# gsanya/orbslam2_NMI

Measured on AMD Instinct MI355X. Metric: pose-candidate NMI evals/sec (640x480, 256 bins), one blocking nmi_search_grid call per step incl. its 8-byte read-back (SURVEY.md 8d's definition); beside the W warm-up steps an untimed clock warm-up of clock_warmup_ms = 200 ms precedes the timed region, higher is better.
Workload: dtype u8

## Files before the change

orbslam2_nmi_amd/csrc/nmi_grid_device.h:

```cpp
#pragma once
#include <hip/hip_runtime.h>
#include <stdint.h>

#include "nmi_kernels.h"
#include "nmi_device.h"

namespace nmi {

namespace {

constexpr int kBlock = NMI_BLOCK_THREADS;
constexpr int kWaves = kBlock / 64;
constexpr int kBins = 256;
constexpr int kWords = kBins * kBins / 2;
constexpr int kRowStride = 129;
constexpr int kJointWords = kBins * kRowStride;
constexpr int kOvfCap = 1024;
constexpr int kRowsPerWave = kBins / kWaves;
constexpr int kLdsTable = 4096;
constexpr int kSide = 8;


struct Lds {
    uint32_t joint[kJointWords];
// ... 30 lines not shown
template <bool BG, bool SHIFTED>
__device__ __forceinline__ void add_pixel(Lds &lds, int par, uint32_t d1, uint32_t d2, int shift)
{
    if (!BG && (d1 == 0 || d2 == 0)) return;
    if (SHIFTED) {
        d1 >>= shift;
        d2 >>= shift;
    }
    const uint32_t word = joint_word(d1, d2), val = joint_inc(d2);
    const uint32_t old = __hip_atomic_fetch_add(&lds.joint[word], val, __ATOMIC_RELAXED, __HIP_MEMORY_SCOPE_WORKGROUP);
    const uint32_t field = val * 0xFFFFu;
    if (__builtin_expect((old & field) == field, 0)) record_wrap(lds, par, word, val, old);
}

__device__ __forceinline__ bool side_add(Lds &lds, int par, uint32_t d1, uint32_t d2, uint32_t weight)
{
    const uint32_t key1 = ((d1 << 8) | d2) + 1u;
    for (int e = 0; e < kSide; ++e) {
        const uint32_t old = atomicCAS(&lds.side_key[par][e], 0u, key1);
        if (old == 0u || old == key1) {
            atomicAdd(&lds.side_cnt[par][e], weight);
            return true;
        }
    }
    return false;
}

template <bool BG, bool SHIFTED, int HIST>
__device__ __forceinline__ bool fold_flat_chunk(Lds &lds, int par, const uint32_t (&r)[4], const uint32_t (&w)[4], int shift)
{
    const uint32_t rb = r[0] & 0xFFu, wb = w[0] & 0xFFu;
    const bool flat = r[0] == r[1] && r[1] == r[2] && r[2] == r[3] && w[0] == w[1] && w[1] == w[2] && w[2] == w[3] &&
                      r[0] == rb * 0x01010101u && w[0] == wb * 0x01010101u;
    if (!__all(flat)) return false;
    uint32_t d1 = rb, d2 = wb;
    const bool skip = !BG && (d1 == 0 || d2 == 0);
    if (SHIFTED) {
        d1 >>= shift;
        d2 >>= shift;
    }
    const uint32_t key = (d1 << 8) | d2;
    const uint32_t key0 = __builtin_amdgcn_readfirstlane(key);
    const bool skip0 = __builtin_amdgcn_readfirstlane((uint32_t)skip) != 0;
    const uint32_t word = joint_word(d1, d2), high = d2 >> 7;
    uint32_t weight = 16;
    bool issue = !skip;
    if (__all(key == key0 && skip == skip0)) {
        const unsigned long long active = __ballot(1);
        weight = 16u * (uint32_t)__popcll(active);
        issue = issue && (__lane_id() == (uint32_t)__ffsll((long long)active) - 1u);
        if (issue && side_add(lds, par, d1, d2, weight)) issue = false;
    }
    if (issue) {
        const uint32_t inc = high ? weight << 16 : weight;
        if (HIST == 2) {
            (void)__hip_atomic_fetch_add(&lds.joint[word], inc, __ATOMIC_RELAXED, __HIP_MEMORY_SCOPE_WORKGROUP);
        } else {
            const uint32_t old = __hip_atomic_fetch_add(&lds.joint[word], inc, __ATOMIC_RELAXED, __HIP_MEMORY_SCOPE_WORKGROUP);
            const uint32_t field_old = high ? old >> 16 : old & 0xFFFFu;
            if (field_old + weight > 0xFFFFu) record_wrap(lds, par, word, high ? 0x10000u : 1u, high ? old : (old | 0xFFFFu));
        }
    }
    return true;
}

template <bool BG, bool SHIFTED, int HIST, bool FOLD>
__device__ __forceinline__ void add_chunk(Lds &lds, int par, const uint4 &rv, const uint4 &wv, int shift, bool try_flat)
{
    const uint32_t r[4] = {rv.x, rv.y, rv.z, rv.w};
    const uint32_t w[4] = {wv.x, wv.y, wv.z, wv.w};
    if (HIST == 0) {
#pragma unroll
        for (int q = 0; q < 4; ++q)
#pragma unroll
            for (int j = 0; j < 4; ++j)
                add_pixel<BG, SHIFTED>(lds, par, (r[q] >> (8 * j)) & 0xFFu, (w[q] >> (8 * j)) & 0xFFu, shift);
        return;
    }
    if (FOLD && HIST != 0 && try_flat) {
        if (__builtin_expect(flat_hint(rv, wv), 0)) {
            if (fold_flat_chunk<BG, SHIFTED, HIST>(lds, par, r, w, shift)) return;
        }
    }
    if (HIST == 2 && BG && !SHIFTED) {
        char *const base = reinterpret_cast<char *>(lds.joint);
        const uint32_t row_bytes = kRowStride * 4, k_ffff = 0xFFFFu;
#pragma unroll
        for (int q = 0; q < 4; ++q) {
#pragma unroll
            for (int j = 0; j < 4; ++j) {
                uint32_t a1, c, addr, hi, val;
                if (j == 0)
                    asm("v_mul_u32_u24_sdwa %0, %1, %2 dst_sel:DWORD dst_unused:UNUSED_PAD src0_sel:BYTE_0 src1_sel:DWORD" : "=v"(a1) : "v"(r[q]), "s"(row_bytes));
                else if (j == 1)
                    asm("v_mul_u32_u24_sdwa %0, %1, %2 dst_sel:DWORD dst_unused:UNUSED_PAD src0_sel:BYTE_1 src1_sel:DWORD" : "=v"(a1) : "v"(r[q]), "s"(row_bytes));
                else if (j == 2)
                    asm("v_mul_u32_u24_sdwa %0, %1, %2 dst_sel:DWORD dst_unused:UNUSED_PAD src0_sel:BYTE_2 src1_sel:DWORD" : "=v"(a1) : "v"(r[q]), "s"(row_bytes));
                else
                    asm("v_mul_u32_u24_sdwa %0, %1, %2 dst_sel:DWORD dst_unused:UNUSED_PAD src0_sel:BYTE_3 src1_sel:DWORD" : "=v"(a1) : "v"(r[q]), "s"(row_bytes));
                c = __builtin_amdgcn_ubfe(w[q], 8 * j, 7);
                asm("v_lshl_add_u32 %0, %1, 2, %2" : "=v"(addr) : "v"(c), "v"(a1));
                hi = __builtin_amdgcn_ubfe(w[q], 8 * j + 7, 1);
                asm("v_mad_u32_u24 %0, %1, %2, 1" : "=v"(val) : "v"(hi), "s"(k_ffff));
                (void)__hip_atomic_fetch_add(reinterpret_cast<uint32_t *>(base + addr), val, __ATOMIC_RELAXED, __HIP_MEMORY_SCOPE_WORKGROUP);
            }
        }
        return;
    }
    uint32_t old[16];
    uint32_t any = 0;
#pragma unroll
    for (int q = 0; q < 4; ++q) {
#pragma unroll
// ... 13 lines not shown
                    old[q * 4 + j] = __hip_atomic_fetch_add(&lds.joint[word], val, __ATOMIC_RELAXED, __HIP_MEMORY_SCOPE_WORKGROUP);
            }
        }
    }
    if (HIST == 1) {
#pragma unroll
        for (int q = 0; q < 4; ++q)
#pragma unroll
            for (int j = 0; j < 4; ++j) {
                uint32_t d2 = (w[q] >> (8 * j)) & 0xFFu;
                if (SHIFTED) d2 >>= shift;
                const uint32_t notfield = (d2 & 128u) ? 0x0000FFFFu : 0xFFFF0000u;
                const uint32_t t = old[q * 4 + j] | notfield;
                any = t > any ? t : any;
            }
        if (__builtin_expect(any == 0xFFFFFFFFu, 0)) {
#pragma unroll
            for (int q = 0; q < 4; ++q)
#pragma unroll
                for (int j = 0; j < 4; ++j) {
                    uint32_t d1 = (r[q] >> (8 * j)) & 0xFFu, d2 = (w[q] >> (8 * j)) & 0xFFu;
                    const bool skip = !BG && (d1 == 0 || d2 == 0);
                    if (SHIFTED) {
                        d1 >>= shift;
                        d2 >>= shift;
                    }
                    const uint32_t val = joint_inc(d2), field = val * 0xFFFFu;
                    if (!skip && (old[q * 4 + j] & field) == field) record_wrap(lds, par, joint_word(d1, d2), val, old[q * 4 + j]);
                }
        }
    }
}

#ifndef NMI_SLAB_SHARES_QUALIFIER
#define NMI_SLAB_SHARES_QUALIFIER __constant__ const
#endif
NMI_SLAB_SHARES_QUALIFIER uint32_t slab_cum[2][kWaves + 1] = {
    {0, 7048, 14096, 21145, 28193, 34369, 40546, 46722, 52899, 55010, 57120, 59231, 61342, 62390, 63439, 64487, 65536},
    {0, 5934, 12896, 19858, 26820, 33147, 39384, 45621, 51859, 54448, 56633, 58818, 61003, 62222, 63327, 64431, 65536},
};

template <bool BG, bool SHIFTED, int HIST, int NT, bool FOLD = true, bool ROWS = false, bool SLABS = false>
__device__ __forceinline__ void histogram_phase(Lds &lds, int par, const GridArgs &a, const uint8_t *__restrict__ render,
                                                const uint8_t *__restrict__ warped, int tid, int c_first, int c_end, bool later = false)
{
    static_assert(!SLABS || NT == kBlock, "slabs are per wavefront of a whole workgroup");
    if (ROWS || a.vec_ok) {
        const int nchunks = c_end;
        const int row_rem = ROWS ? a.width - (a.chunks_per_row << 4) : 0;
        auto ldw = [&](int c) {
            if (ROWS) return *reinterpret_cast<const uint4 *>(warped + (((uint32_t)c << 4) + (uint32_t)__mul24((int)__umulhi((uint32_t)c, a.cpr_magic), row_rem)));
            return *reinterpret_cast<const uint4 *>(warped + ((uint32_t)c << 4));
        };
        auto ldr = [&](int c) {
            const int y = (int)__umulhi((uint32_t)c, a.cpr_magic);
            if (ROWS) {
                const int ry = a.flip ? a.height - 1 - y : y;
                return *reinterpret_cast<const uint4 *>(render + (((uint32_t)(__mul24(y, a.flip_row) + c + a.flip_base) << 4) + (uint32_t)__mul24(ry, row_rem)));
            }
            return *reinterpret_cast<const uint4 *>(render + ((uint32_t)(__mul24(y, a.flip_row) + c + a.flip_base) << 4));
        };
        constexpr bool kHint = FOLD && HIST != 0;
        const bool try_flat = kHint && !(a.phase_mask & 4);
        constexpr int kStep = SLABS ? 64 : NT;
        int base = c_first, stop = nchunks, first = c_first + tid;
        if (SLABS) {
            const uint32_t v = __builtin_amdgcn_readfirstlane((uint32_t)tid >> 6), n = (uint32_t)(nchunks - c_first);
            const uint32_t *cum = slab_cum[later ? 1 : 0];
            base = c_first + (int)(((unsigned long long)n * cum[v]) >> 16);
            stop = c_first + (int)(((unsigned long long)n * cum[v + 1]) >> 16);
            first = base + (tid & 63);
        }
        const int last = SLABS ? max(stop, c_first + 1) - 1 : nchunks - 1;
        const int iters = (stop - base + kStep - 1) / kStep;
        int resume = (HIST == 1 && kHint) ? first : -1;
        if (resume < 0) {
            int ch = first;
            int c0 = min(ch, last);
            uint4 wa = ldw(c0), ra = ldr(c0), wb, rb;
            for (int it = 0; it < iters; it += 2) {
                const int c1 = min(ch + kStep, last);
                wb = ldw(c1);
                rb = ldr(c1);
                if (kHint && __builtin_expect(flat_hint(ra, wa), 0)) {
                    resume = ch;
                    break;
                }
                if (ch < stop) add_chunk<BG, SHIFTED, HIST, false>(lds, par, ra, wa, a.shift, false);
                const int c2 = min(ch + 2 * kStep, last);
                wa = ldw(c2);
                ra = ldr(c2);
                if (kHint && __builtin_expect(flat_hint(rb, wb), 0)) {
                    resume = ch + kStep;
                    break;
                }
                if (ch + kStep < stop) add_chunk<BG, SHIFTED, HIST, false>(lds, par, rb, wb, a.shift, false);
                ch += 2 * kStep;
            }
        }
        if (resume >= 0) {
            int c = min(resume, last);
            uint4 wc = ldw(c), rc = ldr(c);
#pragma unroll 1
            for (int ch = resume; ch < stop; ch += kStep) {
                const int cn = min(ch + kStep, last);
                const uint4 wn = ldw(cn), rn = ldr(cn);
                add_chunk<BG, SHIFTED, HIST, true>(lds, par, rc, wc, a.shift, try_flat);
                wc = wn;
                rc = rn;
            }
        }
        if (ROWS && row_rem > 0) {
            const int x0 = a.chunks_per_row << 4, n = a.height * row_rem;
            for (int t = tid; t < n; t += NT) {
                const int y = t / row_rem, x = x0 + t - y * row_rem;
                const int ry = a.flip ? (a.height - 1 - y) : y;
                uint32_t d1 = render[ry * a.width + x], d2 = warped[y * a.width + x];
                if (HIST == 2) {
                    if (BG || (d1 != 0 && d2 != 0)) {
                        if (SHIFTED) {
                            d1 >>= a.shift;
                            d2 >>= a.shift;
                        }
                        (void)__hip_atomic_fetch_add(&lds.joint[joint_word(d1, d2)], joint_inc(d2), __ATOMIC_RELAXED, __HIP_MEMORY_SCOPE_WORKGROUP);
                    }
                } else {
                    add_pixel<BG, SHIFTED>(lds, par, d1, d2, a.shift);
                }
            }
        }
    } else {
        for (int pos = tid; pos < a.npix; pos += NT) {
            const int y = pos / a.width;
            const int x = pos - y * a.width;
            const int ry = a.flip ? (a.height - 1 - y) : y;
            if (HIST == 2) {
                uint32_t d1 = render[ry * a.width + x], d2 = warped[pos];
                if (BG || (d1 != 0 && d2 != 0)) {
                    if (SHIFTED) {
                        d1 >>= a.shift;
                        d2 >>= a.shift;
                    }
                    (void)__hip_atomic_fetch_add(&lds.joint[joint_word(d1, d2)], joint_inc(d2), __ATOMIC_RELAXED,
// ... 11 lines not shown
    return c ? table[c] : 0.0f;
}
__device__ __forceinline__ float term_lds(const Lds &lds, const float *__restrict__ table, uint32_t c)
{
    float t = lds.table[c < (uint32_t)kLdsTable ? c : 0u];
    if (__builtin_expect(c >= (uint32_t)kLdsTable, 0)) t = table[c];
    return t;
}

static_assert(kWaves == 16 && (kWaves * kRowStride) % 32 == 16, "rows kWaves apart must fall on opposite halves of the 32 banks");
__device__ __forceinline__ int decode_row(int wave, int pass, int r) { return wave + 4 * kWaves * pass + kWaves * r; }
__device__ __forceinline__ bool in_decode_pass(uint32_t d1, int wave, int pass)
{
    return (d1 % (uint32_t)kWaves) == (uint32_t)wave && (d1 / (uint32_t)(4 * kWaves)) == (uint32_t)pass;
}
__device__ __forceinline__ uint32_t decode_word(int d1, int i, int k) { return (uint32_t)(d1 * kRowStride + i + 16 * k); }

__device__ __forceinline__ void apply_wraps(const Lds &lds, int par, uint32_t novf, uint32_t word, uint32_t &lo,
                                            uint32_t &hi)
{
    for (uint32_t e = 0; e < novf; ++e) {
        const uint32_t ev = lds.ovf[par][e];
        if ((ev >> 1) == word) {
            if (ev & 1u) {
                hi += 65536u;
            } else {
                lo += 65536u;
                hi -= 1u;
            }
        }
    }
}

template <bool ZERO0 = false, bool KEPT = false>
__device__ __forceinline__ void decode_phase(Lds &lds, int par, const GridArgs &a, int wave, int lane)
{
    const uint32_t novf = lds.ovf_n[par] < (uint32_t)kOvfCap ? lds.ovf_n[par] : (uint32_t)kOvfCap;
    const bool side_any = lds.side_key[par][0] != 0u;
    uint32_t wave_total = 0;
    const int i = lane & 15, r = lane >> 4;
    uint32_t col_lo[8], col_hi[8];
#pragma unroll
    for (int k = 0; k < 8; ++k) col_lo[k] = col_hi[k] = 0;
#pragma unroll 1
    for (int pass = 0; pass < kRowsPerWave / 4; ++pass) {
        const int d1 = decode_row(wave, pass, r);
        const uint32_t a0 = decode_word(d1, i, 0);
        uint32_t lo[8], hi[8];
#pragma unroll
        for (int k = 0; k < 8; ++k) {
            const uint32_t idx = a0 + 16 * k;
            const uint32_t wd = lds.joint[idx];
            lds.joint[idx] = 0;
            lo[k] = wd & 0xFFFFu;
            hi[k] = wd >> 16;
        }
        if (__builtin_expect(novf != 0, 0)) {
#pragma unroll
            for (int k = 0; k < 8; ++k) apply_wraps(lds, par, novf, a0 + 16 * k, lo[k], hi[k]);
        }
        if (__builtin_expect(side_any, 0)) {
            for (int e = 0; e < kSide; ++e) {
                const uint32_t key1 = __builtin_amdgcn_readfirstlane(lds.side_key[par][e]);
                if (key1 == 0u) break;
                const uint32_t sd1 = (key1 - 1u) >> 8, sd2 = (key1 - 1u) & 0xFFu;
                if (!in_decode_pass(sd1, wave, pass)) continue;
                const uint32_t sword = joint_word(sd1, sd2);
                const uint32_t cnt = lds.side_cnt[par][e];
#pragma unroll
                for (int k = 0; k < 8; ++k) {
                    if (a0 + 16 * k == sword) {
                        if (sd2 & 128u)
                            hi[k] += cnt;
                        else
                            lo[k] += cnt;
                    }
                }
            }
        }
        uint32_t rsum = 0, cmax = 0;
        if (ZERO0) {
            uint32_t raw = 0;
#pragma unroll
            for (int k = 0; k < 8; ++k) raw += lo[k] + hi[k];
            wave_total += row_sum_16(raw);
            if (i == 0) lo[0] = 0;
            if (d1 == 0) {
#pragma unroll
                for (int k = 0; k < 8; ++k) lo[k] = hi[k] = 0;
            }
        }
        float tl[8], th[8];
#pragma unroll
        for (int k = 0; k < 8; ++k) {
            if (!KEPT) {
                col_lo[k] += lo[k];
                col_hi[k] += hi[k];
            }
            rsum += lo[k] + hi[k];
            cmax = max(cmax, max(lo[k], hi[k]));
            tl[k] = lds.table[lo[k] & (kLdsTable - 1)];
            th[k] = lds.table[hi[k] & (kLdsTable - 1)];
        }
        if (__builtin_expect(cmax >= (uint32_t)kLdsTable, 0)) {
#pragma unroll
            for (int k = 0; k < 8; ++k) {
                if (lo[k] >= (uint32_t)kLdsTable) tl[k] = a.table[lo[k]];
                if (hi[k] >= (uint32_t)kLdsTable) th[k] = a.table[hi[k]];
            }
        }
        rsum = row_sum_16(rsum);
        if (!ZERO0) wave_total += rsum;
        const float x = row_tree_16(lane_tree_16(tl, th));
        if (i == 0) {
            lds.hist_render[d1] = rsum;
            lds.joint_row_sums[d1] = x;
        }
        if (a.dbg_joint) {
            uint32_t *row = a.dbg_joint + d1 * kBins;
#pragma unroll
            for (int k = 0; k < 8; ++k) {
                const int q = i + 16 * k;
                row[q] = lo[k];
                row[q + 128] = hi[k];
            }
        }
    }
    if (!KEPT) {
#pragma unroll
        for (int k = 0; k < 8; ++k) {
            const int q = i + 16 * k;
            atomicAdd(&lds.hist_warped[q], col_lo[k]);
            atomicAdd(&lds.hist_warped[q + 128], col_hi[k]);
        }
    }
    if (i == 0) atomicAdd(&lds.total[par], wave_total);
}

__device__ __forceinline__ void final_phase(Lds &lds, const GridArgs &a, int lane, int p, int w, int s,
                                            unsigned long long &prev_key, bool kept = false, float *frame_sum = nullptr)
{
    const int i = lane & 15, r = lane >> 4;
    float lo[8], hi[8];
    const uint32_t *h = r == 0 ? lds.hist_render : lds.hist_warped;
    uint32_t cl[8], ch[8];
#pragma unroll
    for (int k = 0; k < 8; ++k) {
        cl[k] = r < (kept ? 1 : 2) ? h[i + 16 * k] : 0u;
        ch[k] = r < (kept ? 1 : 2) ? h[i + 16 * k + 128] : 0u;
    }
#pragma unroll
    for (int k = 0; k < 8; ++k) {
        lo[k] = a.table[cl[k]];
        hi[k] = a.table[ch[k]];
    }
    if ((w == 0 || s == 0) && a.plan) {
        uint32_t m = 0;
#pragma unroll
        for (int k = 0; k < 8; ++k) m |= (cl[k] != 0u ? 1u << k : 0u) | (ch[k] != 0u ? 0x100u << k : 0u);
        if (lane < 32 && m) __hip_atomic_fetch_or(const_cast<uint32_t *>(&a.plan->seen[lane]), m, __ATOMIC_RELAXED, __HIP_MEMORY_SCOPE_AGENT);
    }
    if (r == 2) {
#pragma unroll
        for (int k = 0; k < 8; ++k) {
            lo[k] = lds.joint_row_sums[i + 16 * k];
            hi[k] = lds.joint_row_sums[i + 16 * k + 128];
        }
    }
    const float x = row_tree_16(lane_tree_16(lo, hi));
// ... 25 lines not shown
    uint32_t bits = 0;
    unsigned long long *post = nullptr;
    uint32_t state = 0, max_joint = 0;
    if (lane == 0) final_key = __hip_atomic_load(a.key, __ATOMIC_RELAXED, __HIP_MEMORY_SCOPE_AGENT);
    if (plan && lane < 32) bits = __hip_atomic_exchange(&plan->seen[lane], 0u, __ATOMIC_RELAXED, __HIP_MEMORY_SCOPE_AGENT);
    if (plan && lane == 0) post = plan->seen_post, state = plan->seen_state, max_joint = plan->seen_max_joint;
    if (lane == 0) {
        __hip_atomic_store(a.done, 0u, __ATOMIC_RELAXED, __HIP_MEMORY_SCOPE_AGENT);
        if (a.out_key) __hip_atomic_store(a.out_key, final_key, __ATOMIC_RELAXED, __HIP_MEMORY_SCOPE_SYSTEM);
        if (a.mailbox)
            __hip_atomic_store(&a.mailbox->word, final_key | ((unsigned long long)(a.seq & 1u) << 63), __ATOMIC_RELAXED, __HIP_MEMORY_SCOPE_SYSTEM);
    }
    if (plan) {
        const uint32_t n = row_sum_16((uint32_t)__popc(bits));
        const uint32_t nw = (uint32_t)__shfl((int)n, 16, 64);
        const uint32_t few = (n > 0u && nw > 0u && n * nw <= max_joint) ? 1u : 0u;
        if (lane == 0 && post && few != state) {
            plan->seen_state = few;
            const uint32_t stamp = 0x80000000u | (uint32_t)wall_clock64();
            __hip_atomic_store(post, ((unsigned long long)stamp << 32) | ((unsigned long long)n << 16) | nw, __ATOMIC_RELAXED, __HIP_MEMORY_SCOPE_SYSTEM);
        }
    }
}

template <bool SHIFTED, bool BG = true, bool ROWS = false>
__device__ __forceinline__ void exact_candidate(Lds &lds, const GridArgs &a, int tid, int p, unsigned long long &prev_key)
{
    const int lane = tid & 63, wave = tid >> 6;
    const int w = p / a.S_local, s = p - w * a.S_local;
    __syncthreads();
    histogram_phase<true, SHIFTED, 1, kBlock, true, ROWS>(lds, 0, a, a.render_stack + (size_t)s * a.npix, a.warp_stack + (size_t)w * a.npix, tid, 0,
                                                          ROWS ? a.height * a.chunks_per_row : a.npix >> 4);
    __syncthreads();
    decode_phase<!BG>(lds, 0, a, wave, lane);
    __syncthreads();
    if (wave == 0) {
        final_phase(lds, a, lane, p, w, s, prev_key);
        for (int t = lane; t < kBins; t += 64) lds.hist_warped[t] = 0;
        if (lane == 0) lds.ovf_n[0] = lds.total[0] = 0;
        if (lane < kSide) lds.side_key[0][lane] = lds.side_cnt[0][lane] = 0;
    }
    __syncthreads();
}

}

}
```

orbslam2_nmi_amd/csrc/nmi_kernels.hip:

```cpp
#include <hip/hip_runtime.h>
#include <stdint.h>

#include "nmi_grid_device.h"

namespace nmi {

#if defined(NMI_GRID_KERNEL_GATED)
#define NMI_GRID_KERNEL_NAME nmi_grid_kernel_gated
#elif defined(NMI_GRID_KERNEL_STAMPED)
#define NMI_GRID_KERNEL_NAME nmi_grid_kernel_stamped
#elif defined(NMI_GRID_KERNEL_ROWS)
#define NMI_GRID_KERNEL_NAME nmi_grid_kernel_rows
#else
#define NMI_GRID_KERNEL_NAME nmi_grid_kernel
#endif
#ifdef NMI_GRID_KERNEL_STAMPED
#define NMI_GRID_STAMP(k)                                                                                         \
    do {                                                                                                          \
        if (a.dbg_stamps && tid == ((k) == 7 ? 64 : 0) && stamp_on) a.dbg_stamps[blockIdx.x * 8 + (k)] = wall_clock64(); \
    } while (0)
#else
#define NMI_GRID_STAMP(k) \
    do {                  \
    } while (0)
// ... 64 lines not shown
    const int slot = slot_in_round(blockIdx.x, gridDim.x);
    int ordinal = slot;
    for (; ordinal < total; ordinal += gridDim.x, par ^= 1) {
        const int p = candidate_at(a, ordinal);
        const int w = p / a.S_local;
        const int s = p - w * a.S_local;
        const uint8_t *render = a.render_stack + (size_t)s * a.npix;
        const uint8_t *warped = a.warp_stack + (size_t)w * a.npix;
#ifdef NMI_GRID_KERNEL_STAMPED
        stamp_on = ordinal == stamp_ordinal;
#endif
        NMI_GRID_STAMP(7);

        if (a.phase_mask & 1) {
            if (a.phase_mask & 8) {
                if (wave < kWaves / 2) histogram_phase<kCountAll, SHIFTED, kFirst, kBlock / 2, true, kRows>(lds, par, a, render, warped, tid, 0, NMI_ALL_CHUNKS);
            } else
                histogram_phase<kCountAll, SHIFTED, kFirst, kBlock, true, kRows, kSlabs>(lds, par, a, render, warped, tid, 0, NMI_ALL_CHUNKS, ordinal != slot);
        }
        if (table_pending) {
#pragma unroll
            for (int k = 0; k < kLdsTable / kBlock; ++k) lds.table[tid + k * kBlock] = tab[k];
            table_pending = false;
        }
        NMI_GRID_STAMP(2);
#ifdef NMI_GRID_KERNEL_STAMPED
        if (a.dbg_stamps && lane == 0 && stamp_on) a.dbg_stamps[gridDim.x * 8 + blockIdx.x * 16 + wave] = wall_clock64();
#endif
        __syncthreads();
        NMI_GRID_STAMP(3);
        const bool kept = keep_ok && w == kept_w && !(s == 0 && a.plan);
        if (a.phase_mask & 2) {
            if (kKeepWarp && kept) decode_phase<false, true>(lds, par, a, wave, lane);
            else decode_phase<kZero0>(lds, par, a, wave, lane);
        }
        kept_w = w;
        __syncthreads();
        NMI_GRID_STAMP(4);
        if (kOptimistic && (a.phase_mask & 3) == 3 && lds.total[par] != (uint32_t)a.npix) {
            exact_from = ordinal;
            break;
        }
        if (wave == 0) {
            if (a.phase_mask & 2) final_phase(lds, a, lane, p, w, s, prev_key, kept, kKeepWarp ? &frame_sum : nullptr);
            if (!kept)
                for (int t = lane; t < kBins; t += 64) lds.hist_warped[t] = 0;
            if (lane == 0) {
                lds.ovf_n[par] = 0;
                lds.total[par ^ 1] = 0;
            }
            if (lane < kSide) {
                int l = lane;
                asm volatile("" : "+v"(l));
                lds.side_key[par][l] = lds.side_cnt[par][l] = 0;
            }
        }
        NMI_GRID_STAMP(5);
    }

    if (kOptimistic && exact_from >= 0) {
        __syncthreads();
        if (tid < kBins) lds.hist_warped[tid] = 0;
        if (tid < 2) lds.total[tid] = lds.ovf_n[tid] = 0;
        if (tid < 2 * kSide) (&lds.side_key[0][0])[tid] = (&lds.side_cnt[0][0])[tid] = 0;
        __syncthreads();
        for (int o = exact_from; o < total; o += gridDim.x) exact_candidate<SHIFTED, !kZero0, kRows>(lds, a, tid, candidate_at(a, o), prev_key);
    }

    if (wave == 0 && !(a.phase_mask & 16)) {
        finish_search(a, lane, prev_key, gridDim.x);
    }
#ifdef NMI_GRID_KERNEL_STAMPED
    stamp_on = true;
#endif
    NMI_GRID_STAMP(6);
}

// ... 337 lines not shown
```

orbslam2_nmi_amd/csrc/nmi_device.h:

```cpp
#pragma once
#include <hip/hip_runtime.h>
#include <stdint.h>

#include "nmi_kernels.h"

namespace nmi {
namespace {

template <int N>
__device__ __forceinline__ float row_shl(float x)
{
    return __builtin_bit_cast(float, __builtin_amdgcn_update_dpp(0, __builtin_bit_cast(int, x), 0x100 + N, 0xF, 0xF, true));
}
template <int N>
__device__ __forceinline__ uint32_t row_shl(uint32_t x)
{
    return (uint32_t)__builtin_amdgcn_update_dpp(0, (int)x, 0x100 + N, 0xF, 0xF, true);
}
__device__ __forceinline__ float row_tree_16(float x)
{
    x = x + row_shl<8>(x);
    x = x + row_shl<4>(x);
    x = x + row_shl<2>(x);
    x = x + row_shl<1>(x);
    return x;
}
__device__ __forceinline__ uint32_t row_sum_16(uint32_t x)
{
    x += row_shl<8>(x);
    x += row_shl<4>(x);
    x += row_shl<2>(x);
    x += row_shl<1>(x);
    return x;
}
__device__ __forceinline__ float lane_tree_16(const float (&lo)[8], const float (&hi)[8])
{
    float s[8];
#pragma unroll
    for (int k = 0; k < 8; ++k) s[k] = lo[k] + hi[k];
#pragma unroll
    for (int k = 0; k < 4; ++k) s[k] = s[k] + s[k + 4];
    s[0] = s[0] + s[2];
    s[1] = s[1] + s[3];
    return s[0] + s[1];
}

__device__ __forceinline__ bool flat_hint(const uint4 &rv, const uint4 &wv)
{
    unsigned long long m;
    asm volatile("v_cmp_eq_u32 vcc, %1, %2\n\tv_cmp_eq_u32 %0, %3, %4\n\ts_and_b64 %0, %0, vcc"
                 : "=s"(m)
                 : "v"(rv.x), "v"(rv.w), "v"(wv.x), "v"(wv.w)
                 : "vcc");
    return m == __builtin_amdgcn_read_exec();
}

__device__ __forceinline__ void commit_score(const GridArgs &a, int p, int w, int s, float a1, float a2, float a3,
                                             unsigned long long &prev_key)
{
    float score;
    if (a1 == 0.0f && a2 == 0.0f && a3 == 0.0f)
        score = 0.0f;
    else if (a.mode == NMI_MODE_ENMI_)
        score = ((-a1) + (-a2)) / (-a3);
    else if (a.mode == NMI_MODE_SUC_)
        score = 2.0f * (1.0f - ((-a3) / ((-a1) + (-a2))));
    else
        score = -1.0f;
    if (a.ratings) a.ratings[p] = score;
    if (a.dbg_sums) {
        a.dbg_sums[0] = a1;
        a.dbg_sums[1] = a2;
        a.dbg_sums[2] = a3;
    }
    if (a.score_post)
        __hip_atomic_store(a.score_post, (unsigned long long)__float_as_uint(score) | ((unsigned long long)a.seq << 32),
                           __ATOMIC_RELAXED, __HIP_MEMORY_SCOPE_SYSTEM);
    if (score >= 0.0f) {
        const uint32_t bits = score == 0.0f ? 0u : __float_as_uint(score);
        const uint32_t gidx = (uint32_t)(a.w_offset + w) * (uint32_t)a.S_total + (uint32_t)(a.s_offset + s);
        const unsigned long long key = ((unsigned long long)bits << 32) | (unsigned long long)(0xFFFFFFFFu - gidx);
        prev_key = __hip_atomic_fetch_max(a.key, key, __ATOMIC_RELAXED, __HIP_MEMORY_SCOPE_AGENT);
    }
}

__device__ __forceinline__ bool publish_winner(const GridArgs &a, unsigned long long prev_key)
{
    const unsigned int one = prev_key == ~0ull ? 2u : 1u;
// ... 17 lines not shown
```

orbslam2_nmi_amd/csrc/nmi_pix_device.h:

```cpp
#pragma once
#include <hip/hip_runtime.h>
#include <stdint.h>

#include <type_traits>

#include "nmi_grid_device.h"
#include "nmi_mask_device.h"

namespace nmi {

namespace {

typedef uint32_t u32x4 __attribute__((ext_vector_type(4)));

constexpr int kUnits = kWords / 4;
constexpr int kUnitsPerLane = kUnits / kBlock;
constexpr int kGranules = kWaves * kUnitsPerLane * 2;
struct PixHeader {
    unsigned long long granule[kGranules];
    uint32_t side_key[kSide];
    uint32_t side_cnt[kSide];
    uint32_t pad[16];
};
static_assert(sizeof(PixHeader) == 2048 + 128 && sizeof(PixHeader) % 128 == 0, "whole lines");
// ... 103 lines not shown
__device__ __forceinline__ uint32_t add_row_tails(Lds &lds, const Pieces &pc, const uint8_t *__restrict__ render, const uint8_t *__restrict__ warped, Take take)
{
    const GridArgs &a = pc.a;
    uint32_t added = 0;
    if (pc.d.off == 0 && pc.row_rem > 0) {
        const int x0 = a.chunks_per_row << 4, n = a.height * pc.row_rem;
        for (int t = pc.wave * 64 + pc.lane; t < n; t += kBlock) {
            const int y = t / pc.row_rem, x = x0 + t - y * pc.row_rem;
            const int pos = y * a.width + x, rpos = (a.flip ? a.height - 1 - y : y) * a.width + x;
            if (!take(pos, rpos)) continue;
            uint32_t d1 = render[rpos], d2 = warped[pos];
            if (SHIFTED) {
                d1 >>= a.shift;
                d2 >>= a.shift;
            }
            (void)__hip_atomic_fetch_add(&lds.joint[joint_word(d1, d2)], joint_inc(d2), __ATOMIC_RELAXED, __HIP_MEMORY_SCOPE_WORKGROUP);
            ++added;
        }
    }
    return added;
}

template <bool SHIFTED>
__device__ __forceinline__ void histogram_dealt(Lds &lds, const GridArgs &a, const uint8_t *__restrict__ render, const uint8_t *__restrict__ warped,
                                                int wave, int lane, const Deal &d)
{
    const Pieces pc(a, d, wave, lane);
    auto ldw = [&](int c) { return ld16(warped, pc.at(c)); };
    auto ldr = [&](int c) { return ld16(render, pc.rat(c)); };
    const int nchunks = pc.nchunks, iters = pc.iters();
    (void)add_row_tails<SHIFTED>(lds, pc, render, warped, [](int, int) { return true; });
    if (iters <= 0) return;
    const bool try_flat = !(a.phase_mask & 4);
    int resume = -1;
    int c = pc.chunk_of(0);
    uint4 wa = ldw(c), ra = ldr(c), wb, rb;
    for (int it = 0; it < iters; it += 2) {
        const int cb = pc.chunk_of(it + 1);
        wb = ldw(cb);
        rb = ldr(cb);
        if (__builtin_expect(flat_hint(ra, wa), 0)) {
            resume = it;
            break;
        }
        if (c < nchunks) add_chunk<true, SHIFTED, 2, false>(lds, 0, ra, wa, a.shift, false);
        c = pc.chunk_of(it + 2);
        wa = ldw(c);
        ra = ldr(c);
        if (__builtin_expect(flat_hint(rb, wb), 0)) {
            resume = it + 1;
            break;
        }
        if (cb < nchunks) add_chunk<true, SHIFTED, 2, false>(lds, 0, rb, wb, a.shift, false);
    }
    if (resume >= 0) {
        int cc = pc.chunk_of(resume);
        uint4 wc = ldw(cc), rc = ldr(cc);
#pragma unroll 1
        for (int it = resume; it < iters; ++it) {
            const int cn = pc.chunk_of(it + 1);
            const uint4 wn = ldw(cn), rn = ldr(cn);
            if (cc < nchunks) add_chunk<true, SHIFTED, 2, true>(lds, 0, rc, wc, a.shift, try_flat);
            wc = wn;
            rc = rn;
            cc = cn;
        }
    }
}

__device__ __forceinline__ uint32_t mask_popc(const uint4 &m)
{
    return __popc(nonzero_byte_bits(m.x)) + __popc(nonzero_byte_bits(m.y)) + __popc(nonzero_byte_bits(m.z)) + __popc(nonzero_byte_bits(m.w));
}

template <bool SHIFTED, bool COVERED>
__device__ __forceinline__ uint32_t masked_histogram_dealt(Lds &lds, const GridArgs &a, const uint8_t *__restrict__ render,
                                                          const uint8_t *__restrict__ warped, const uint8_t *__restrict__ wmask,
                                                          const uint8_t *__restrict__ rmask, int wave, int lane, const Deal &d)
{
    const Pieces pc(a, d, wave, lane);
    uint32_t added = add_row_tails<SHIFTED>(lds, pc, render, warped, [&](int pos, int rpos) { return wmask[pos] != 0 && (!COVERED || rmask[rpos] != 0); });
    const int iters = pc.iters();
    if (iters <= 0) return added;
    int c = pc.chunk_of(0);
    uint32_t o = pc.at(c), ro = pc.rat(c);
    uint4 wc = ld16(warped, o), rc = ld16(render, ro), mc = ld16(wmask, o);
    if (COVERED) mc = both_nonzero(mc, ld16(rmask, ro));
#pragma unroll 1
    for (int it = 0; it < iters; ++it) {
        const int cn = pc.chunk_of(it + 1);
        o = pc.at(cn);
        ro = pc.rat(cn);
        const uint4 wn = ld16(warped, o), rn = ld16(render, ro), wmn = ld16(wmask, o), rmn = COVERED ? ld16(rmask, ro) : wmn;
        if (c < pc.nchunks) {
            added += COVERED ? popc4(mc) : mask_popc(mc);
            masked_add_chunk<true, SHIFTED, 2>(lds, 0, rc, wc, mc, a.shift);
        }
        wc = wn;
        rc = rn;
// ... 301 lines not shown
```

Measured before the change: 9.481 million.

## Add lean packed-halves decode path using udot2 for sums and table addressing

Splits the decode phase into a lean fast path and the original full path. When a pass has no overflow wraps, no side entries and all 16-bit halves stay below 4096, the lean path skips unpacking. It sums packed words with udot2, accumulates packed column counts, and computes LDS table addresses directly with udot2. Otherwise it falls back to decode_pass_full, which now does per-pass atomic column adds. The aim is to cut ALU work in the decode loop, at the cost of extra ballot checks, more code, and risk of packed-column overflow across passes.

```diff
diff --git a/orbslam2_nmi_amd/csrc/nmi_grid_device.h b/orbslam2_nmi_amd/csrc/nmi_grid_device.h
--- a/orbslam2_nmi_amd/csrc/nmi_grid_device.h
+++ b/orbslam2_nmi_amd/csrc/nmi_grid_device.h
@@ -366,82 +366,85 @@
     }
 }
 
-template <bool ZERO0 = false, bool KEPT = false>
-__device__ __forceinline__ void decode_phase(Lds &lds, int par, const GridArgs &a, int wave, int lane)
-{
+typedef unsigned short PackedHalves __attribute__((ext_vector_type(2)));
+__device__ __forceinline__ uint32_t halves_dot(uint32_t word, uint32_t weights, uint32_t acc)
+{
+    return __builtin_amdgcn_udot2(__builtin_bit_cast(PackedHalves, word), __builtin_bit_cast(PackedHalves, weights), acc, false);
+}
+typedef __attribute__((address_space(3))) const float LdsTerm;
+__device__ __forceinline__ uint32_t lds_byte_address(const void *p) { return (uint32_t)(uintptr_t)p; }
+__device__ __forceinline__ float lds_term_at(uint32_t byte_address) { return *(LdsTerm *)(uintptr_t)byte_address; }
+
+template <bool ZERO0, bool KEPT>
+__device__ __forceinline__ void decode_pass_full(Lds &lds, int par, const GridArgs &a, int wave, int pass, int i, int d1, uint32_t a0,
+                                                 uint32_t novf, bool side_any, const uint32_t (&wd)[8], uint32_t &rsum,
+                                                 uint32_t &wave_total, float (&tl)[8], float (&th)[8]);
+
+template <bool ZERO0 = false, bool KEPT = false, bool LEAN = true>
+__device__ __forceinline__ void decode_phase(Lds &lds, int par, const GridArgs &a, int wave_of_lane, int lane)
+{
+    const int wave = __builtin_amdgcn_readfirstlane(wave_of_lane);
     const uint32_t novf = lds.ovf_n[par] < (uint32_t)kOvfCap ? lds.ovf_n[par] : (uint32_t)kOvfCap;
     const bool side_any = lds.side_key[par][0] != 0u;
+    uint32_t full_passes = __builtin_amdgcn_readfirstlane((novf != 0u || a.dbg_joint) ? 0xFu : 0u);
+    if (__builtin_expect(__builtin_amdgcn_readfirstlane(side_any ? 1 : 0) != 0, 0)) {
+        for (int e = 0; e < kSide; ++e) {
+            const uint32_t key1 = __builtin_amdgcn_readfirstlane(lds.side_key[par][e]);
+            if (key1 == 0u) break;
+            const uint32_t sd1 = (key1 - 1u) >> 8;
+            if ((sd1 % (uint32_t)kWaves) == (uint32_t)wave) full_passes |= 1u << (sd1 / (uint32_t)(4 * kWaves));
+        }
+    }
+    const uint32_t table_at = lds_byte_address(lds.table);
     uint32_t wave_total = 0;
     const int i = lane & 15, r = lane >> 4;
-    uint32_t col_lo[8], col_hi[8];
-#pragma unroll
-    for (int k = 0; k < 8; ++k) col_lo[k] = col_hi[k] = 0;
+    uint32_t col[8];
+#pragma unroll
+    for (int k = 0; k < 8; ++k) col[k] = 0;
 #pragma unroll 1
     for (int pass = 0; pass < kRowsPerWave / 4; ++pass) {
         const int d1 = decode_row(wave, pass, r);
         const uint32_t a0 = decode_word(d1, i, 0);
-        uint32_t lo[8], hi[8];
+        uint32_t wd[8];
 #pragma unroll
         for (int k = 0; k < 8; ++k) {
             const uint32_t idx = a0 + 16 * k;
-            const uint32_t wd = lds.joint[idx];
+            wd[k] = lds.joint[idx];
             lds.joint[idx] = 0;
-            lo[k] = wd & 0xFFFFu;
-            hi[k] = wd >> 16;
-        }
-        if (__builtin_expect(novf != 0, 0)) {
-#pragma unroll
-            for (int k = 0; k < 8; ++k) apply_wraps(lds, par, novf, a0 + 16 * k, lo[k], hi[k]);
-        }
-        if (__builtin_expect(side_any, 0)) {
-            for (int e = 0; e < kSide; ++e) {
-                const uint32_t key1 = __builtin_amdgcn_readfirstlane(lds.side_key[par][e]);
-                if (key1 == 0u) break;
-                const uint32_t sd1 = (key1 - 1u) >> 8, sd2 = (key1 - 1u) & 0xFFu;
-                if (!in_decode_pass(sd1, wave, pass)) continue;
-                const uint32_t sword = joint_word(sd1, sd2);
-                const uint32_t cnt = lds.side_cnt[par][e];
-#pragma unroll
-                for (int k = 0; k < 8; ++k) {
-                    if (a0 + 16 * k == sword) {
-                        if (sd2 & 128u)
-                            hi[k] += cnt;
-                        else
-                            lo[k] += cnt;
-                    }
-                }
-            }
-        }
-        uint32_t rsum = 0, cmax = 0;
-        if (ZERO0) {
-            uint32_t raw = 0;
-#pragma unroll
-            for (int k = 0; k < 8; ++k) raw += lo[k] + hi[k];
-            wave_total += row_sum_16(raw);
-            if (i == 0) lo[0] = 0;
-            if (d1 == 0) {
-#pragma unroll
-                for (int k = 0; k < 8; ++k) lo[k] = hi[k] = 0;
-            }
-        }
+        }
+        const uint32_t any = (wd[0] | wd[1] | wd[2]) | (wd[3] | wd[4] | wd[5]) | (wd[6] | wd[7]);
+        uint32_t rsum = 0;
         float tl[8], th[8];
-#pragma unroll
-        for (int k = 0; k < 8; ++k) {
-            if (!KEPT) {
-                col_lo[k] += lo[k];
-                col_hi[k] += hi[k];
-            }
-            rsum += lo[k] + hi[k];
-            cmax = max(cmax, max(lo[k], hi[k]));
-            tl[k] = lds.table[lo[k] & (kLdsTable - 1)];
-            th[k] = lds.table[hi[k] & (kLdsTable - 1)];
-        }
-        if (__builtin_expect(cmax >= (uint32_t)kLdsTable, 0)) {
+        if (LEAN && __builtin_expect(((full_passes >> pass) & 1u) == 0u && __builtin_amdgcn_ballot_w64((any & 0xF000F000u) != 0u) == 0ull, 1)) {
+            rsum = halves_dot((wd[0] + wd[1] + wd[2]) + (wd[3] + wd[4]) + (wd[5] + wd[6]) + wd[7], 0x00010001u, 0u);
+            if (ZERO0) {
+                wave_total += row_sum_16(rsum);
+                if (i == 0) {
+                    rsum -= wd[0] & 0xFFFFu;
+                    wd[0] &= 0xFFFF0000u;
+                }
+                if (d1 == 0) {
+                    rsum = 0;
+#pragma unroll
+                    for (int k = 0; k < 8; ++k) wd[k] = 0;
+                }
+            }
+            uint32_t at[16];
 #pragma unroll
             for (int k = 0; k < 8; ++k) {
-                if (lo[k] >= (uint32_t)kLdsTable) tl[k] = a.table[lo[k]];
-                if (hi[k] >= (uint32_t)kLdsTable) th[k] = a.table[hi[k]];
-            }
+                if (!KEPT) col[k] += wd[k];
+                at[k] = halves_dot(wd[k], 0x00000004u, table_at);
+                at[k + 8] = halves_dot(wd[k], 0x00040000u, table_at);
+            }
+            asm volatile("" : "+v"(at[0]), "+v"(at[1]), "+v"(at[2]), "+v"(at[3]), "+v"(at[4]), "+v"(at[5]), "+v"(at[6]), "+v"(at[7]),
+                              "+v"(at[8]), "+v"(at[9]), "+v"(at[10]), "+v"(at[11]), "+v"(at[12]), "+v"(at[13]), "+v"(at[14]), "+v"(at[15]));
+#pragma unroll
+            for (int k = 0; k < 8; ++k) {
+                tl[k] = lds_term_at(at[k]);
+                th[k] = lds_term_at(at[k + 8]);
+            }
+        } else {
+            decode_pass_full<ZERO0, KEPT>(lds, par, a, wave, pass, i, d1, a0, novf, side_any, wd, rsum, wave_total, tl, th);
         }
         rsum = row_sum_16(rsum);
         if (!ZERO0) wave_total += rsum;
@@ -450,25 +453,93 @@
             lds.hist_render[d1] = rsum;
             lds.joint_row_sums[d1] = x;
         }
-        if (a.dbg_joint) {
-            uint32_t *row = a.dbg_joint + d1 * kBins;
-#pragma unroll
-            for (int k = 0; k < 8; ++k) {
-                const int q = i + 16 * k;
-                row[q] = lo[k];
-                row[q + 128] = hi[k];
-            }
-        }
     }
     if (!KEPT) {
 #pragma unroll
         for (int k = 0; k < 8; ++k) {
             const int q = i + 16 * k;
-            atomicAdd(&lds.hist_warped[q], col_lo[k]);
-            atomicAdd(&lds.hist_warped[q + 128], col_hi[k]);
+            atomicAdd(&lds.hist_warped[q], col[k] & 0xFFFFu);
+            atomicAdd(&lds.hist_warped[q + 128], col[k] >> 16);
         }
     }
     if (i == 0) atomicAdd(&lds.total[par], wave_total);
+}
+
+template <bool ZERO0, bool KEPT>
+__device__ __forceinline__ void decode_pass_full(Lds &lds, int par, const GridArgs &a, int wave, int pass, int i, int d1, uint32_t a0,
+                                                 uint32_t novf, bool side_any, const uint32_t (&wd)[8], uint32_t &rsum,
+                                                 uint32_t &wave_total, float (&tl)[8], float (&th)[8])
+{
+    uint32_t lo[8], hi[8];
+#pragma unroll
+    for (int k = 0; k < 8; ++k) {
+        lo[k] = wd[k] & 0xFFFFu;
+        hi[k] = wd[k] >> 16;
+    }
+    if (__builtin_expect(novf != 0, 0)) {
+#pragma unroll
+        for (int k = 0; k < 8; ++k) apply_wraps(lds, par, novf, a0 + 16 * k, lo[k], hi[k]);
+    }
+    if (__builtin_expect(side_any, 0)) {
+        for (int e = 0; e < kSide; ++e) {
+            const uint32_t key1 = __builtin_amdgcn_readfirstlane(lds.side_key[par][e]);
+            if (key1 == 0u) break;
+            const uint32_t sd1 = (key1 - 1u) >> 8, sd2 = (key1 - 1u) & 0xFFu;
+            if (!in_decode_pass(sd1, wave, pass)) continue;
+            const uint32_t sword = joint_word(sd1, sd2);
+            const uint32_t cnt = lds.side_cnt[par][e];
+#pragma unroll
+            for (int k = 0; k < 8; ++k) {
+                if (a0 + 16 * k == sword) {
+                    if (sd2 & 128u)
+                        hi[k] += cnt;
+                    else
+                        lo[k] += cnt;
+                }
+            }
+        }
+    }
+    uint32_t cmax = 0;
+    rsum = 0;
+    if (ZERO0) {
+        uint32_t raw = 0;
+#pragma unroll
+        for (int k = 0; k < 8; ++k) raw += lo[k] + hi[k];
+        wave_total += row_sum_16(raw);
+        if (i == 0) lo[0] = 0;
+        if (d1 == 0) {
+#pragma unroll
+            for (int k = 0; k < 8; ++k) lo[k] = hi[k] = 0;
+        }
+    }
+#pragma unroll
+    for (int k = 0; k < 8; ++k) {
+        if (!KEPT) {
+            const int q = i + 16 * k;
+            atomicAdd(&lds.hist_warped[q], lo[k]);
+            atomicAdd(&lds.hist_warped[q + 128], hi[k]);
+        }
+        rsum += lo[k] + hi[k];
+        cmax = max(cmax, max(lo[k], hi[k]));
+        tl[k] = lds.table[lo[k] & (kLdsTable - 1)];
+        th[k] = lds.table[hi[k] & (kLdsTable - 1)];
+    }
+    if (__builtin_expect(cmax >= (uint32_t)kLdsTable, 0)) {
+#pragma unroll
+        for (int k = 0; k < 8; ++k) {
+            if (lo[k] >= (uint32_t)kLdsTable) tl[k] = a.table[lo[k]];
+            if (hi[k] >= (uint32_t)kLdsTable) th[k] = a.table[hi[k]];
+        }
+    }
+    if (a.dbg_joint) {
+        uint32_t *row = a.dbg_joint + d1 * kBins;
+#pragma unroll
+        for (int k = 0; k < 8; ++k) {
+            const int q = i + 16 * k;
+            row[q] = lo[k];
+            row[q + 128] = hi[k];
+        }
+    }
 }
 
 __device__ __forceinline__ void final_phase(Lds &lds, const GridArgs &a, int lane, int p, int w, int s,
@@ -560,10 +631,12 @@
     histogram_phase<true, SHIFTED, 1, kBlock, true, ROWS>(lds, 0, a, a.render_stack + (size_t)s * a.npix, a.warp_stack + (size_t)w * a.npix, tid, 0,
                                                           ROWS ? a.height * a.chunks_per_row : a.npix >> 4);
     __syncthreads();
-    decode_phase<!BG>(lds, 0, a, wave, lane);
+    decode_phase<!BG, false, false>(lds, 0, a, wave, lane);
     __syncthreads();
     if (wave == 0) {
-        final_phase(lds, a, lane, p, w, s, prev_key);
+        int l = lane;
+        asm volatile("" : "+v"(l));
+        final_phase(lds, a, l, p, w, s, prev_key);
         for (int t = lane; t < kBins; t += 64) lds.hist_warped[t] = 0;
         if (lane == 0) lds.ovf_n[0] = lds.total[0] = 0;
         if (lane < kSide) lds.side_key[0][lane] = lds.side_cnt[0][lane] = 0;
diff --git a/orbslam2_nmi_amd/csrc/nmi_kernels.hip b/orbslam2_nmi_amd/csrc/nmi_kernels.hip
--- a/orbslam2_nmi_amd/csrc/nmi_kernels.hip
+++ b/orbslam2_nmi_amd/csrc/nmi_kernels.hip
@@ -120,7 +120,7 @@
         const bool kept = keep_ok && w == kept_w && !(s == 0 && a.plan);
         if (a.phase_mask & 2) {
             if (kKeepWarp && kept) decode_phase<false, true>(lds, par, a, wave, lane);
-            else decode_phase<kZero0>(lds, par, a, wave, lane);
+            else decode_phase<kZero0, false, kOptimistic>(lds, par, a, wave, lane);
         }
         kept_w = w;
         __syncthreads();
@@ -130,7 +130,9 @@
             break;
         }
         if (wave == 0) {
-            if (a.phase_mask & 2) final_phase(lds, a, lane, p, w, s, prev_key, kept, kKeepWarp ? &frame_sum : nullptr);
+            int l = lane;
+            if (!kOptimistic) asm volatile("" : "+v"(l));
+            if (a.phase_mask & 2) final_phase(lds, a, l, p, w, s, prev_key, kept, kKeepWarp ? &frame_sum : nullptr);
             if (!kept)
                 for (int t = lane; t < kBins; t += 64) lds.hist_warped[t] = 0;
             if (lane == 0) {
```

After: 9.541 million (median of 6 runs). Within noise of the previous version (+0.6%).

## Fold partially flat waves and return to fast path after flat runs

Applied to the files above, without the earlier changes.

The flat-region fold now works on the subset of lanes holding identical flat chunks instead of requiring the whole wave to be flat. The switch to the careful loop fires once at least a threshold of in-range lanes are flat. The loop also drops back to the unrolled fast loop once a chunk is no longer hot. Slab split boundaries are retuned as well. The aim is to collapse more repeated LDS atomics in large uniform image areas without staying in the slower careful loop for the rest of the pass. The cost is extra ballots and readlanes per chunk and more complex control flow.

```diff
diff --git a/orbslam2_nmi_amd/csrc/nmi_device.h b/orbslam2_nmi_amd/csrc/nmi_device.h
--- a/orbslam2_nmi_amd/csrc/nmi_device.h
+++ b/orbslam2_nmi_amd/csrc/nmi_device.h
@@ -45,15 +45,32 @@
     return s[0] + s[1];
 }
 
-__device__ __forceinline__ bool flat_hint(const uint4 &rv, const uint4 &wv)
+__device__ __forceinline__ unsigned long long flat_mask(const uint4 &rv, const uint4 &wv)
 {
     unsigned long long m;
     asm volatile("v_cmp_eq_u32 vcc, %1, %2\n\tv_cmp_eq_u32 %0, %3, %4\n\ts_and_b64 %0, %0, vcc"
                  : "=s"(m)
                  : "v"(rv.x), "v"(rv.w), "v"(wv.x), "v"(wv.w)
                  : "vcc");
-    return m == __builtin_amdgcn_read_exec();
+    return m;
 }
+__device__ __forceinline__ bool flat_hint(const uint4 &rv, const uint4 &wv) { return flat_mask(rv, wv) == __builtin_amdgcn_read_exec(); }
+
+#ifndef NMI_FLAT_TRIGGER
+#define NMI_FLAT_TRIGGER 8
+#endif
+constexpr int kFlatTrigger = NMI_FLAT_TRIGGER;
+__device__ __forceinline__ bool flat_trigger(const uint4 &rv, const uint4 &wv, unsigned long long lanes)
+{
+    unsigned long long m;
+    int n;
+    asm volatile("v_cmp_eq_u32 vcc, %2, %3\n\tv_cmp_eq_u32 %0, %4, %5\n\ts_and_b64 %0, %0, vcc\n\ts_and_b64 %0, %0, %6\n\ts_bcnt1_i32_b64 %1, %0"
+                 : "=&s"(m), "=s"(n)
+                 : "v"(rv.x), "v"(rv.w), "v"(wv.x), "v"(wv.w), "s"(lanes)
+                 : "vcc", "scc");
+    return n >= kFlatTrigger;
+}
+__device__ __forceinline__ unsigned long long first_lanes(int n) { return n >= 64 ? ~0ull : n <= 0 ? 0ull : (1ull << n) - 1ull; }
 
 __device__ __forceinline__ void commit_score(const GridArgs &a, int p, int w, int s, float a1, float a2, float a3,
                                              unsigned long long &prev_key)
diff --git a/orbslam2_nmi_amd/csrc/nmi_grid_device.h b/orbslam2_nmi_amd/csrc/nmi_grid_device.h
--- a/orbslam2_nmi_amd/csrc/nmi_grid_device.h
+++ b/orbslam2_nmi_amd/csrc/nmi_grid_device.h
@@ -86,23 +86,24 @@
     const uint32_t rb = r[0] & 0xFFu, wb = w[0] & 0xFFu;
     const bool flat = r[0] == r[1] && r[1] == r[2] && r[2] == r[3] && w[0] == w[1] && w[1] == w[2] && w[2] == w[3] &&
                       r[0] == rb * 0x01010101u && w[0] == wb * 0x01010101u;
-    if (!__all(flat)) return false;
+    const unsigned long long flat_lanes = __ballot(flat);
+    if (flat_lanes == 0) return false;
     uint32_t d1 = rb, d2 = wb;
     const bool skip = !BG && (d1 == 0 || d2 == 0);
     if (SHIFTED) {
         d1 >>= shift;
         d2 >>= shift;
     }
-    const uint32_t key = (d1 << 8) | d2;
-    const uint32_t key0 = __builtin_amdgcn_readfirstlane(key);
-    const bool skip0 = __builtin_amdgcn_readfirstlane((uint32_t)skip) != 0;
+    const uint32_t key = (d1 << 8) | d2 | (skip ? 0x10000u : 0u);
+    const uint32_t key0 = (uint32_t)__builtin_amdgcn_readlane((int)key, __ffsll((long long)flat_lanes) - 1);
+    const bool same = flat && key == key0;
+    const unsigned long long same_lanes = __ballot(same);
     const uint32_t word = joint_word(d1, d2), high = d2 >> 7;
     uint32_t weight = 16;
-    bool issue = !skip;
-    if (__all(key == key0 && skip == skip0)) {
-        const unsigned long long active = __ballot(1);
-        weight = 16u * (uint32_t)__popcll(active);
-        issue = issue && (__lane_id() == (uint32_t)__ffsll((long long)active) - 1u);
+    bool issue = flat && !skip;
+    if (same) {
+        weight = 16u * (uint32_t)__popcll(same_lanes);
+        issue = issue && (__lane_id() == (uint32_t)__ffsll((long long)same_lanes) - 1u);
         if (issue && side_add(lds, par, d1, d2, weight)) issue = false;
     }
     if (issue) {
@@ -115,7 +116,7 @@
             if (field_old + weight > 0xFFFFu) record_wrap(lds, par, word, high ? 0x10000u : 1u, high ? old : (old | 0xFFFFu));
         }
     }
-    return true;
+    return flat;
 }
 
 template <bool BG, bool SHIFTED, int HIST, bool FOLD>
@@ -132,7 +133,7 @@
         return;
     }
     if (FOLD && HIST != 0 && try_flat) {
-        if (__builtin_expect(flat_hint(rv, wv), 0)) {
+        if (flat_mask(rv, wv) != 0) {
             if (fold_flat_chunk<BG, SHIFTED, HIST>(lds, par, r, w, shift)) return;
         }
     }
@@ -212,12 +213,15 @@
     }
 }
 
+#ifndef NMI_FLAT_RETURN
+#define NMI_FLAT_RETURN 1
+#endif
 #ifndef NMI_SLAB_SHARES_QUALIFIER
 #define NMI_SLAB_SHARES_QUALIFIER __constant__ const
 #endif
 NMI_SLAB_SHARES_QUALIFIER uint32_t slab_cum[2][kWaves + 1] = {
-    {0, 7048, 14096, 21145, 28193, 34369, 40546, 46722, 52899, 55010, 57120, 59231, 61342, 62390, 63439, 64487, 65536},
-    {0, 5934, 12896, 19858, 26820, 33147, 39384, 45621, 51859, 54448, 56633, 58818, 61003, 62222, 63327, 64431, 65536},
+    {0, 6141, 13058, 19975, 26893, 33023, 39154, 45284, 51415, 54172, 56688, 59205, 61722, 62790, 63705, 64621, 65536},
+    {0, 5741, 12554, 19367, 26180, 32321, 38461, 44601, 50742, 53676, 56275, 58875, 61475, 62604, 63582, 64559, 65536},
 };
 
 template <bool BG, bool SHIFTED, int HIST, int NT, bool FOLD = true, bool ROWS = false, bool SLABS = false>
@@ -253,42 +257,54 @@
         }
         const int last = SLABS ? max(stop, c_first + 1) - 1 : nchunks - 1;
         const int iters = (stop - base + kStep - 1) / kStep;
-        int resume = (HIST == 1 && kHint) ? first : -1;
-        if (resume < 0) {
-            int ch = first;
-            int c0 = min(ch, last);
-            uint4 wa = ldw(c0), ra = ldr(c0), wb, rb;
-            for (int it = 0; it < iters; it += 2) {
-                const int c1 = min(ch + kStep, last);
-                wb = ldw(c1);
-                rb = ldr(c1);
-                if (kHint && __builtin_expect(flat_hint(ra, wa), 0)) {
-                    resume = ch;
-                    break;
+        const int lane0 = SLABS ? base : c_first + (int)__builtin_amdgcn_readfirstlane((uint32_t)tid & ~63u);
+        auto in_range = [&](int it) { return first_lanes(stop - lane0 - it * kStep); };
+        bool careful = HIST == 1 && kHint;
+        constexpr bool kReturn = NMI_FLAT_RETURN != 0 && HIST != 1;
+        for (int it = 0;;) {
+            int ch = first + it * kStep;
+            if (!careful) {
+                int c0 = min(ch, last);
+                uint4 wa = ldw(c0), ra = ldr(c0), wb, rb;
+                for (; it < iters; it += 2) {
+                    const int c1 = min(ch + kStep, last);
+                    wb = ldw(c1);
+                    rb = ldr(c1);
+                    if (kHint && __builtin_expect(flat_trigger(ra, wa, in_range(it)), 0)) {
+                        careful = true;
+                        break;
+                    }
+                    if (ch < stop) add_chunk<BG, SHIFTED, HIST, false>(lds, par, ra, wa, a.shift, false);
+                    const int c2 = min(ch + 2 * kStep, last);
+                    wa = ldw(c2);
+                    ra = ldr(c2);
+                    if (kHint && __builtin_expect(flat_trigger(rb, wb, in_range(it + 1)), 0)) {
+                        careful = true;
+                        ++it;
+                        ch += kStep;
+                        break;
+                    }
+                    if (ch + kStep < stop) add_chunk<BG, SHIFTED, HIST, false>(lds, par, rb, wb, a.shift, false);
+                    ch += 2 * kStep;
                 }
-                if (ch < stop) add_chunk<BG, SHIFTED, HIST, false>(lds, par, ra, wa, a.shift, false);
-                const int c2 = min(ch + 2 * kStep, last);
-                wa = ldw(c2);
-                ra = ldr(c2);
-                if (kHint && __builtin_expect(flat_hint(rb, wb), 0)) {
-                    resume = ch + kStep;
-                    break;
-                }
-                if (ch + kStep < stop) add_chunk<BG, SHIFTED, HIST, false>(lds, par, rb, wb, a.shift, false);
-                ch += 2 * kStep;
-            }
-        }
-        if (resume >= 0) {
-            int c = min(resume, last);
+                if (!careful) break;
+            }
+            int c = min(ch, last);
             uint4 wc = ldw(c), rc = ldr(c);
 #pragma unroll 1
-            for (int ch = resume; ch < stop; ch += kStep) {
+            while (it < iters) {
                 const int cn = min(ch + kStep, last);
                 const uint4 wn = ldw(cn), rn = ldr(cn);
-                add_chunk<BG, SHIFTED, HIST, true>(lds, par, rc, wc, a.shift, try_flat);
+                const bool hot = !kReturn || flat_trigger(rc, wc, in_range(it));
+                if (ch < stop) add_chunk<BG, SHIFTED, HIST, true>(lds, par, rc, wc, a.shift, try_flat);
                 wc = wn;
                 rc = rn;
-            }
+                ch += kStep;
+                ++it;
+                if (!hot) break;
+            }
+            if (it >= iters) break;
+            careful = false;
         }
         if (ROWS && row_rem > 0) {
             const int x0 = a.chunks_per_row << 4, n = a.height * row_rem;
diff --git a/orbslam2_nmi_amd/csrc/nmi_pix_device.h b/orbslam2_nmi_amd/csrc/nmi_pix_device.h
--- a/orbslam2_nmi_amd/csrc/nmi_pix_device.h
+++ b/orbslam2_nmi_amd/csrc/nmi_pix_device.h
@@ -159,39 +159,49 @@
     (void)add_row_tails<SHIFTED>(lds, pc, render, warped, [](int, int) { return true; });
     if (iters <= 0) return;
     const bool try_flat = !(a.phase_mask & 4);
-    int resume = -1;
-    int c = pc.chunk_of(0);
-    uint4 wa = ldw(c), ra = ldr(c), wb, rb;
-    for (int it = 0; it < iters; it += 2) {
-        const int cb = pc.chunk_of(it + 1);
-        wb = ldw(cb);
-        rb = ldr(cb);
-        if (__builtin_expect(flat_hint(ra, wa), 0)) {
-            resume = it;
-            break;
-        }
-        if (c < nchunks) add_chunk<true, SHIFTED, 2, false>(lds, 0, ra, wa, a.shift, false);
-        c = pc.chunk_of(it + 2);
-        wa = ldw(c);
-        ra = ldr(c);
-        if (__builtin_expect(flat_hint(rb, wb), 0)) {
-            resume = it + 1;
-            break;
-        }
-        if (cb < nchunks) add_chunk<true, SHIFTED, 2, false>(lds, 0, rb, wb, a.shift, false);
-    }
-    if (resume >= 0) {
-        int cc = pc.chunk_of(resume);
+    auto in_range = [&](int c) { return first_lanes(nchunks - (int)__builtin_amdgcn_readfirstlane((uint32_t)(c - lane))); };
+    bool careful = false;
+    for (int it = 0;;) {
+        if (!careful) {
+            int c = pc.chunk_of(it);
+            uint4 wa = ldw(c), ra = ldr(c), wb, rb;
+            for (; it < iters; it += 2) {
+                const int cb = pc.chunk_of(it + 1);
+                wb = ldw(cb);
+                rb = ldr(cb);
+                if (__builtin_expect(flat_trigger(ra, wa, in_range(c)), 0)) {
+                    careful = true;
+                    break;
+                }
+                if (c < nchunks) add_chunk<true, SHIFTED, 2, false>(lds, 0, ra, wa, a.shift, false);
+                c = pc.chunk_of(it + 2);
+                wa = ldw(c);
+                ra = ldr(c);
+                if (__builtin_expect(flat_trigger(rb, wb, in_range(cb)), 0)) {
+                    careful = true;
+                    ++it;
+                    break;
+                }
+                if (cb < nchunks) add_chunk<true, SHIFTED, 2, false>(lds, 0, rb, wb, a.shift, false);
+            }
+            if (!careful) break;
+        }
+        int cc = pc.chunk_of(it);
         uint4 wc = ldw(cc), rc = ldr(cc);
 #pragma unroll 1
-        for (int it = resume; it < iters; ++it) {
+        while (it < iters) {
             const int cn = pc.chunk_of(it + 1);
             const uint4 wn = ldw(cn), rn = ldr(cn);
+            const bool hot = NMI_FLAT_RETURN == 0 || flat_trigger(rc, wc, in_range(cc));
             if (cc < nchunks) add_chunk<true, SHIFTED, 2, true>(lds, 0, rc, wc, a.shift, try_flat);
             wc = wn;
             rc = rn;
             cc = cn;
-        }
+            ++it;
+            if (!hot) break;
+        }
+        if (it >= iters) break;
+        careful = false;
     }
 }
 
```

New measurement: 9.486 million before, 9.448 million after. About the same (-0.4%).
